# anton-v-bilan/mpeg1video-decoder-webgl

Hardware: AMD Instinct MI355X
Metric: 1080p macroblocks/s (higher is better)
Workload: dtype int32/u8

## Files before the change

mpeg1video-decoder-webgl_amd/csrc/leon_kernels.h:

```cpp
#pragma once
#include <hip/hip_runtime.h>
#include <stdint.h>
#include "leon_resize_row.h"


namespace leon {

struct PicDesc {
    const int16_t* coef[4];
    const uint8_t* qscale;
    const uint8_t* intra;
    const uint8_t* repadd;
    const uint8_t* mb_dir;
    const int16_t* mv_fwd;
    const int16_t* mv_bwd;
    uint8_t*       out;
    const uint8_t* ref_fwd;
    const uint8_t* ref_bwd;
    int32_t        type;
    uint32_t       n_entries;
    const uint32_t* grp_off;
    const uint32_t* entries;
    uint8_t*       rgba;
    int32_t        no_planes;
// ... 235 lines not shown
    o.p43 = v2f{fy6, fy6} + v2f{fy7, -fy7};
    return o;
}

__device__ __forceinline__ ColOut butterfly8_col(const int (&X)[8], int n_live)
{
    const int c128 = 128;
    if (n_live <= 2) {
        const int X0 = X[0], X1 = X[1];
        int x4 = div256(mad24k(X1, 473, c128)) - X1;
        int x0 = x4 - div256(mad24k(X1, 362, c128));
        int y7 = -x0 - div256(mad24k(X1, 196, c128));
        return col_final(X0, X1, X0, x4, X0, x0, X0, y7);
    } else if (n_live <= 4) {
        const int X0 = X[0], X1 = X[1], X2 = X[2], X3 = X[3];
        int b7 = X1 + X3;
        int x4 = div256(mad24k(X1, 473, mad24k(X3, 196, c128))) - b7;
        int x0 = x4 - div256(mad24k(X1 - X3, 362, c128));
        int x2 = div256(mad24k(X2, 362, c128)) - X2;
        int y7 = -x0 - div256(mad24k(X3, -473, mad24k(X1, 196, c128)));
        return col_final(X0 + X2, b7, X0 + x2, x4, X0 - x2, x0, X0 - X2, y7);
    } else {
        int b1 = X[4];
        int b3 = X[2] + X[6];
        int b4 = X[5] - X[3];
        int tmp1 = X[1] + X[7];
        int tmp2 = X[3] + X[5];
        int b6 = X[1] - X[7];
        int b7 = tmp1 + tmp2;
        int m0 = X[0];
        int x4 = div256(mad24k(b6, 473, mad24k(b4, -196, c128))) - b7;
        int x0 = x4 - div256(mad24k(tmp1 - tmp2, 362, c128));
        int x1 = m0 - b1;
        int x2 = div256(mad24k(X[2] - X[6], 362, c128)) - b3;
        int x3 = m0 + b1;
        int y7 = -x0 - div256(mad24k(b4, 473, mad24k(b6, 196, c128)));
        return col_final(x3 + b3, b7, x1 + x2, x4, x1 - x2, x0, x3 - b3, y7);
    }
}

__device__ __forceinline__ int dequant_any(int X, int qO, int pm, int nim, int lo2048, int hi2047)
{
    const int sg = sign3(X);
    int x2 = (X << 1) + (sg & nim);
    int t = mul24_asm(x2, qO);
    int f = t >> 4;
    int z;
    asm("v_med3_i32 %0, %1, 0, 1" : "=v"(z) : "v"(f));
    f = (f - z) | (sg & 1);
    asm("v_med3_i32 %0, %1, %2, %3" : "=v"(f) : "v"(f), "s"(lo2048), "v"(hi2047));
    return __mul24(f, pm);
}

__device__ __forceinline__ int cvt_floor(float x)
{
    int d;
    asm("v_cvt_flr_i32_f32 %0, %1" : "=v"(d) : "v"(x));
    return d;
}

__device__ __forceinline__ int handoff16(int w)
{
    int r = (int)(short)w;
    if (w >= 65536) r = (w & 255) - 256;
    if (w < -65536) r = w & 255;
    return r;
}


__device__ __forceinline__ uint32_t avg4_u8x4(uint32_t a, uint32_t b, uint32_t c, uint32_t d)
{
    const uint32_t X = __builtin_amdgcn_lerp(a, b, c ^ d);
    const uint32_t y = __builtin_amdgcn_lerp(c, d, 0u);
    return __builtin_amdgcn_lerp(X, y, 0x01010101u);
}

__device__ __forceinline__ uint32_t ref_px_clamped(const LEON_GLOBAL uint8_t* ref, uint32_t row_off, int W, int x)
{
    int t = min(max(x >> 2, 0), (W >> 2) - 1);
    return ldg<uint8_t>(ref, row_off + (uint32_t)(4 * t + (x & 3)));
}

typedef v3u U3 __attribute__((aligned(4)));

struct RefRows {
    uint32_t l0, l1, l2;
    uint32_t m0, m1, m2;
    uint32_t s;
    uint32_t oh;
};

__device__ __forceinline__ void gather9_slow(const LEON_GLOBAL uint8_t* ref, uint32_t row_off, int W, int px,
                                             uint32_t& a0, uint32_t& a1, uint32_t& a2)
{
    uint32_t lo = 0, hi = 0;
#pragma unroll 1
    for (int k = 0; k < 4; k++) {
        lo |= ref_px_clamped(ref, row_off, W, px + k) << (8 * k);
        hi |= ref_px_clamped(ref, row_off, W, px + 4 + k) << (8 * k);
    }
    a0 = lo;
    a1 = hi;
    a2 = ref_px_clamped(ref, row_off, W, px + 8);
}

__device__ __forceinline__ int clamp_med3(int v, int hi)
{
    int d;
    asm("v_med3_i32 %0, %1, 0, %2" : "=v"(d) : "v"(v), "s"(hi));
    return d;
}

__device__ __forceinline__ RefRows fetch_rows(const LEON_GLOBAL uint8_t* ref, int W, int H, int y,
                                              int px, int ay, int oh, int ov, bool in_pic, bool last_row, bool use)
{
    const int yy = y + ay;
    const uint32_t r0 = (uint32_t)__mul24(clamp_med3(yy, H - 1), W);
    const uint32_t r1 = r0 + ((uint32_t)yy < (uint32_t)(H - 1) ? (uint32_t)W : 0u);
    RefRows R;
    R.oh = (uint32_t)oh;
    R.m0 = R.m1 = R.m2 = 0;
    if (in_pic) {
        R.s = (uint32_t)px & 3u;
        uint32_t xo = (uint32_t)px & ~3u;
        const __amdgpu_buffer_rsrc_t rs = buf_rsrc((const void*)ref);
        const v3u a = __builtin_amdgcn_raw_buffer_load_b96(rs, (int)(use ? r0 + xo : kOobBit), 0, 0);
        const v3u c = __builtin_amdgcn_raw_buffer_load_b96(rs, (int)(use && last_row && ov ? r1 + xo : kOobBit), 0, 0);
        R.l0 = a.x; R.l1 = a.y; R.l2 = a.z;
        R.m0 = c.x; R.m1 = c.y; R.m2 = c.z;
    } else {
        R.s = 0;
        gather9_slow(ref, r0, W, px, R.l0, R.l1, R.l2);
        if (last_row && ov) gather9_slow(ref, r1, W, px, R.m0, R.m1, R.m2);
    }
    return R;
}

__device__ __forceinline__ void finish_rows(RefRows& R, int ov, bool last_row, int lane, const RefRows* below = nullptr)
{
    const int src = (ov ? ((lane + 8) & 63) : lane) << 2;
    const uint32_t n0 = (uint32_t)__builtin_amdgcn_ds_bpermute(src, (int)R.l0);
    const uint32_t n1 = (uint32_t)__builtin_amdgcn_ds_bpermute(src, (int)R.l1);
    const uint32_t n2 = (uint32_t)__builtin_amdgcn_ds_bpermute(src, (int)R.l2);
    if (below) {
        const uint32_t b0 = (uint32_t)__builtin_amdgcn_ds_bpermute(src, (int)below->l0);
        const uint32_t b1 = (uint32_t)__builtin_amdgcn_ds_bpermute(src, (int)below->l1);
        const uint32_t b2 = (uint32_t)__builtin_amdgcn_ds_bpermute(src, (int)below->l2);
        const bool wrap = last_row && ov;
        R.m0 = wrap ? b0 : n0; R.m1 = wrap ? b1 : n1; R.m2 = wrap ? b2 : n2;
        return;
    }
    if (!(last_row && ov)) { R.m0 = n0; R.m1 = n1; R.m2 = n2; }
}

__device__ __forceinline__ v2u predict8(const RefRows& R)
{
    uint32_t a0 = __builtin_amdgcn_alignbyte(R.l1, R.l0, R.s);
    uint32_t a1 = __builtin_amdgcn_alignbyte(R.l2, R.l1, R.s);
    uint32_t a2 = __builtin_amdgcn_alignbyte(0u, R.l2, R.s);
    uint32_t c0 = __builtin_amdgcn_alignbyte(R.m1, R.m0, R.s);
    uint32_t c1 = __builtin_amdgcn_alignbyte(R.m2, R.m1, R.s);
    uint32_t c2 = __builtin_amdgcn_alignbyte(0u, R.m2, R.s);
    uint32_t b0 = __builtin_amdgcn_alignbyte(a1, a0, R.oh);
    uint32_t b1 = __builtin_amdgcn_alignbyte(a2, a1, R.oh);
    uint32_t d0 = __builtin_amdgcn_alignbyte(c1, c0, R.oh);
    uint32_t d1 = __builtin_amdgcn_alignbyte(c2, c1, R.oh);
    v2u p;
    p.x = avg4_u8x4(a0, b0, c0, d0);
    p.y = avg4_u8x4(a1, b1, c1, d1);
    return p;
}

template <int M>
__device__ __forceinline__ uint32_t pred_x256(uint32_t pred)
{
    uint32_t d;
    asm("v_perm_b32 %0, 0, %1, %2" : "=v"(d) : "v"(pred), "s"(0x0c0c000cu | ((uint32_t)M << 8)));
    return d;
}


struct Display {
    char* stash;
    int side;
    char* apark;
    const char* lut;
    uint8_t* planes;
    const struct FrameOut* fo;
};
static constexpr int kAlphaNone = 0, kAlphaPark = 1, kAlphaTake = 2;

template <int I>
__device__ __forceinline__ uint32_t byte_shl(uint32_t v, uint32_t sh)
{
    uint32_t d;
    if constexpr (I == 0) asm("v_lshlrev_b32_sdwa %0, %1, %2 dst_sel:DWORD dst_unused:UNUSED_PAD src0_sel:DWORD src1_sel:BYTE_0" : "=v"(d) : "v"(sh), "v"(v));
    else if constexpr (I == 1) asm("v_lshlrev_b32_sdwa %0, %1, %2 dst_sel:DWORD dst_unused:UNUSED_PAD src0_sel:DWORD src1_sel:BYTE_1" : "=v"(d) : "v"(sh), "v"(v));
    else if constexpr (I == 2) asm("v_lshlrev_b32_sdwa %0, %1, %2 dst_sel:DWORD dst_unused:UNUSED_PAD src0_sel:DWORD src1_sel:BYTE_2" : "=v"(d) : "v"(sh), "v"(v));
    else asm("v_lshlrev_b32_sdwa %0, %1, %2 dst_sel:DWORD dst_unused:UNUSED_PAD src0_sel:DWORD src1_sel:BYTE_3" : "=v"(d) : "v"(sh), "v"(v));
    return d;
}

struct ChromaTerms { int r, g, b; };
template <int I>
__device__ __forceinline__ ChromaTerms chroma_terms(const char* lut, uint32_t cb2, uint32_t cr2, uint32_t three)
{
    const v2u rc = *reinterpret_cast<const v2u*>(lut + 1024 + byte_shl<I>(cr2, three));
    const v2u bc = *reinterpret_cast<const v2u*>(lut + 3072 + byte_shl<I>(cb2, three));
    return ChromaTerms{(int)rc.x, (int)(rc.y + bc.y), (int)bc.x};
}
template <int I>
__device__ __forceinline__ uint32_t rgba_px(const char* lut, uint32_t y4, const ChromaTerms& c, int a_fixed, uint32_t two)
{
    const int ys = *reinterpret_cast<const int*>(lut + byte_shl<I>(y4, two));
    uint32_t px;
    asm("v_ashr_pk_u8_i32 %0, %1, %2, %3" : "=v"(px) : "v"(ys + c.r), "v"(ys + c.g), "n"(kLutShift));
    asm("v_ashr_pk_u8_i32 %0, %1, %2, %3 op_sel:[0,0,0,1]" : "+v"(px) : "v"(ys + c.b), "v"(a_fixed), "n"(kLutShift));
    return px;
}
template <bool ALPHA>
// ... 50 lines not shown
#pragma unroll
        for (int i = 0; i < 8; i++) o |= *reinterpret_cast<const uint16_t*>(cp + i * 128);
        live[h] = lanes_nonzero((int)o);
        const uint32_t pos = __builtin_amdgcn_mbcnt_hi((uint32_t)(live[h] >> 32), __builtin_amdgcn_mbcnt_lo((uint32_t)live[h], n_before));
        if (o != 0u) *reinterpret_cast<uint8_t*>(ids + pos) = (uint8_t)(tag + (uint32_t)lane + 64u * h);
        n_before += (uint32_t)__builtin_popcountll(live[h]);
    }
    return n_before;
}

template <bool PAIR, bool TLDS = true>
__device__ __forceinline__ void column_pass(char* tile0, uint32_t tile_step, const char* ids, const char* qtab, uint32_t n_cols, int qia0, int qia1, int lane,
                                            uint32_t qreg = 0u)
{
    int lo2048 = -2048, hi2047 = 2047;
    asm("" : "+s"(lo2048), "+v"(hi2047));
#pragma unroll 1
    for (uint32_t base = 0; base < n_cols; base += 64u) {
        const uint32_t k = base + (uint32_t)lane;
        const bool act = k < n_cols;
        uint32_t id = *reinterpret_cast<const uint8_t*>(ids + k);
        id = act ? id : 0u;
        char* colp = tile0 + ((id & 0x47u) << 4) + ((id >> 2) & 14u);
        if constexpr (PAIR) colp += (id >> 7) * tile_step;
        int X[8];
#pragma unroll
        for (int i = 0; i < 8; i++) X[i] = *reinterpret_cast<const short*>(colp + i * 128);
        int bq = __builtin_amdgcn_ds_bpermute((int)((id & 7u) << 2), qia0);
        if constexpr (PAIR) {
            const int bq1 = __builtin_amdgcn_ds_bpermute((int)((id & 7u) << 2), qia1);
            bq = (id & 128u) ? bq1 : bq;
        }
        const bool bia = bq >= 256;
        const uint32_t qv = (uint32_t)bq & 31u;
        v2u msel, pm8;
        if constexpr (TLDS) {
            const char* const qt = qtab + (id & 56u);
            msel = *reinterpret_cast<const v2u*>(qt + (bia ? 0 : 64));
            pm8 = *reinterpret_cast<const v2u*>(qt + 128);
        } else {
            const int qo = (int)((id & 56u) + (bia ? 0u : 64u)), po = (int)((id & 56u) + 128u);
            msel.x = (uint32_t)__builtin_amdgcn_ds_bpermute(qo, (int)qreg);
            msel.y = (uint32_t)__builtin_amdgcn_ds_bpermute(qo + 4, (int)qreg);
            pm8.x = (uint32_t)__builtin_amdgcn_ds_bpermute(po, (int)qreg);
            pm8.y = (uint32_t)__builtin_amdgcn_ds_bpermute(po + 4, (int)qreg);
        }
        int nim = bia ? 0 : -1;
        asm("" : "+v"(nim));
        const bool dc_lane = bia && (id & 56u) == 0u;
        uint64_t nz[8];
#pragma unroll
        for (int i = 0; i < 8; i++) nz[i] = lanes_nonzero(X[i]);
        const int dc = X[0];
        int rows_live = 1;
#pragma unroll
        for (int i = 0; i < 8; i++) {
            if (nz[i] != 0) {
                rows_live = i + 1;
                int P = (int)(((i < 4 ? pm8.x : pm8.y) >> (8 * (i & 3))) & 255u);
                const int qO = (int)__umul24(qv, ((i < 4 ? msel.x : msel.y) >> (8 * (i & 3))) & 255u);
                X[i] = dequant_any(X[i], qO, P, nim, lo2048, hi2047);
            }
        }
        if (dc_lane) X[0] = dc * 256;
        const ColOut co = butterfly8_col(X, rows_live);
        const v2f k04 = {0.4f, 0.4f};
        const v2f s07 = co.p07 * k04, s16 = co.p16 * k04, s52 = co.p52 * k04, s43 = co.p43 * k04;
        int wi[8] = {cvt_floor(s07.x), cvt_floor(s16.x), cvt_floor(s52.y), cvt_floor(s43.y),
                     cvt_floor(s43.x), cvt_floor(s52.x), cvt_floor(s16.y), cvt_floor(s07.y)};
        const float mx = fmaxf(fmaxf(fmaxf(fabsf(s07.x), fabsf(s16.x)), fmaxf(fabsf(s52.y), fabsf(s43.y))),
                               fmaxf(fmaxf(fabsf(s43.x), fabsf(s52.x)), fmaxf(fabsf(s16.y), fabsf(s07.y))));
        if (mx >= 32768.0f) {
#pragma unroll
            for (int n = 0; n < 8; n++) wi[n] = handoff16(wi[n]);
        }
        if (act) {
#pragma unroll
            for (int n = 0; n < 8; n++) *reinterpret_cast<short*>(colp + n * 128) = (short)wi[n];
        }
    }
}

struct MbCarry { uint32_t flags; };
static constexpr int kCarryNone = 0, kCarryLeave = 1, kCarryTake = 2;

template <int TYPE_, bool SPARSE_> struct PlainLuma {
    static constexpr int TYPE = TYPE_, AMODE = kAlphaNone, CARRY = kCarryNone, LAYOUT = 0, OUT = kOutRgba; static constexpr bool SPARSE = SPARSE_, CHROMA = false, DISPLAY = false, BACK = false;
};
template <int TYPE, bool SPARSE> struct PlainChroma : PlainLuma<TYPE, SPARSE> { static constexpr bool CHROMA = true; };
template <int TYPE, bool SPARSE, int LAYOUT_, int OUT_> struct DisplayChroma : PlainChroma<TYPE, SPARSE> {
    static constexpr int CARRY = kCarryLeave, LAYOUT = LAYOUT_, OUT = OUT_; static constexpr bool DISPLAY = true;
};
template <int TYPE, bool SPARSE, int OUT_> struct DisplayLuma : PlainLuma<TYPE, SPARSE> {
    static constexpr int CARRY = kCarryTake, OUT = OUT_; static constexpr bool DISPLAY = true;
};
template <int TYPE, bool SPARSE, int OUT> struct YuvaAPart : DisplayLuma<TYPE, SPARSE, OUT> { static constexpr int AMODE = kAlphaPark; };
template <int TYPE, bool SPARSE, int OUT> struct YuvaYPart : DisplayLuma<TYPE, SPARSE, OUT> { static constexpr int AMODE = kAlphaTake; };
template <int TYPE, int OUT> struct PairBackHalf : DisplayLuma<TYPE, false, OUT> { static constexpr int LAYOUT = 1; static constexpr bool BACK = true; };

struct TaskArgs {
    bool alpha = false;
    char* tile = nullptr;
    uint64_t live[2] = {0, 0};
    uint32_t qreg = 0u;
};

template <int LAYOUT>
__device__ __forceinline__ void column_front(const PicDesc& pd, char* lds, char* tile, int lane, int qia, uint32_t qreg, uint64_t (&live)[2])
{
    const uint32_t n_cols = scan_tile(tile, lds + Lay<LAYOUT>::slots, lane, 0u, 0u, live);
    wave_sync();
    column_pass<false, Lay<LAYOUT>::tables_in_lds>(tile, 0u, lds + Lay<LAYOUT>::slots, Lay<LAYOUT>::tables_in_lds ? lds + kOffQtab : reinterpret_cast<const char*>(pd.qt),
                                                   n_cols, qia, qia, lane, qreg);
    wave_sync();
}

template <typename V>
__device__ __forceinline__ void recon_task(const PicDesc& pd, const Geom& G, int Rt, int g, char* lds, int lane, Display dsp, MbCarry& carry, const TaskArgs& args = TaskArgs())
{
    constexpr int TYPE = V::TYPE, AMODE = V::AMODE, CARRY = V::CARRY, LAYOUT = V::LAYOUT, OUT = V::OUT;
    constexpr bool CHROMA = V::CHROMA, SPARSE = V::SPARSE, DISPLAY = V::DISPLAY, BACK = V::BACK;
    static_assert(!BACK || (LAYOUT == 1 && CARRY == kCarryTake), "a back half runs on the two-tile layout behind the chroma part");
    const bool alpha = AMODE == kAlphaPark || args.alpha;
    char* const tile = BACK ? args.tile : lds;
    const int W = CHROMA ? G.cw >> 1 : G.cw;
    const int H = CHROMA ? G.ch >> 1 : G.ch;
    const int bw = W >> 3;
    const uint32_t ysz = (uint32_t)G.cw * (uint32_t)G.ch;
    const uint32_t a_off = !CHROMA && alpha ? ysz + (ysz >> 1) : 0u;
    const int hi3 = lane >> 3, lo3 = lane & 7;

    const int Qld = g * 8 + lo3;
    const bool ld_ok = Qld < bw;
    const int b = lo3;
    const int Qb = g * 8 + b;
    const bool valid = Qb < bw;
    const int Qs = valid ? Qb : bw - 1;
    const int R0 = CHROMA ? Rt : 2 * Rt;
    const uint32_t coef_voff = (2u * ((uint32_t)__mul24(8 * R0 + hi3, W) + (uint32_t)(8 * Qld))) | (ld_ok ? 0u : kOobBit);
    const uint32_t half_step = CHROMA ? 0u : 8u * (uint32_t)W;
    uint32_t ent_first[2] = {0u, 0u}, ent_start[2] = {0u, 0u}, ent_count[2] = {0u, 0u};
    const __amdgpu_buffer_rsrc_t ent_rs = __builtin_amdgcn_make_buffer_rsrc(
        (void*)(SPARSE ? pd.entries : nullptr), 0, SPARSE ? (int)(pd.n_entries * 4u) : 0, 0x00020000);
    if constexpr (SPARSE) {
        const uint32_t nY = 2u * (uint32_t)G.tasksY, nC = (uint32_t)G.tasksC;
        const uint32_t gid0 = CHROMA ? nY + (uint32_t)(Rt * G.gC + g) : (uint32_t)(2 * Rt * G.gY + g) + (alpha ? nY + 2u * nC : 0u);
        const uint32_t gid1 = CHROMA ? gid0 + nC : gid0 + (uint32_t)G.gY;
        const LEON_GLOBAL uint32_t* go = gptr(pd.grp_off);
        const uint32_t gid[2] = {gid0, gid1};
#pragma unroll
        for (int h = 0; h < 2; h++) {
            const uint32_t s0 = go[gid[h]], e0 = go[gid[h] + 1];
            ent_start[h] = s0;
            ent_count[h] = e0 > s0 ? min(e0 - s0, 512u) : 0u;
            ent_first[h] = (uint32_t)__builtin_amdgcn_raw_buffer_load_b32(
                ent_rs, (int)(((s0 + (uint32_t)lane) * 4u) | ((uint32_t)lane < ent_count[h] ? 0u : kOobBit)), 0, kAuxStreamOnce);
        }
    } else if constexpr (!BACK) {
        wait_lds_all();
        __builtin_amdgcn_wave_barrier();
        coef_rows_to_lds(pd.coef[CHROMA ? 1 : (alpha ? 3 : 0)], lds, coef_voff, 0u);
        coef_rows_to_lds(pd.coef[CHROMA ? 2 : (alpha ? 3 : 0)], lds + kLdsHalf, coef_voff, 2u * half_step);
    }
    const uint32_t mb = (uint32_t)(CHROMA ? Rt * G.mbw + Qs : Rt * G.mbw + (Qs >> 1));
    uint32_t mf = 0, mk = 0, flags;
    if constexpr (CARRY == kCarryTake) {
        const int src = (4 * dsp.side + (lo3 >> 1)) << 2;
        flags = (uint32_t)__builtin_amdgcn_ds_bpermute(src, (int)carry.flags);
        if (TYPE != 1) mf = *reinterpret_cast<const uint32_t*>(lds + Lay<LAYOUT>::carry + src);
        if (TYPE == 3) mk = *reinterpret_cast<const uint32_t*>(lds + Lay<LAYOUT>::carry + 32 + src);
    } else {
        flags = (uint32_t)(ldg<uint8_t>(gptr(pd.qscale), mb) & 31) | (ldg<uint8_t>(gptr(pd.intra), mb) != 0 ? 256u : 0u);
        if (TYPE != 1) {
            flags |= ldg<uint8_t>(gptr(pd.repadd), mb) >= 128 ? 512u : 0u;
            mf = ldg<uint32_t>(gptr(pd.mv_fwd), mb * 4);
        }
        if (TYPE == 3) {
            mk = ldg<uint32_t>(gptr(pd.mv_bwd), mb * 4);
            flags |= (uint32_t)(ldg<uint8_t>(gptr(pd.mb_dir), mb) & 3) << 10;
        }
        if constexpr (CARRY == kCarryLeave) {
            carry.flags = flags;
            if (TYPE != 1) *reinterpret_cast<uint32_t*>(lds + Lay<LAYOUT>::carry + ((lane & 7) << 2)) = mf;
            if (TYPE == 3) *reinterpret_cast<uint32_t*>(lds + Lay<LAYOUT>::carry + 32 + ((lane & 7) << 2)) = mk;
        }
    }
    const int q = (int)(flags & 31u);
    const bool ia = (flags & 256u) != 0u;
    const int x0 = 8 * Qs;
    bool nopred = false;
    int pxA = 0, ayA = 0, ohA = 0, ovA = 0, pxB = 0, ayB = 0, ohB = 0, ovB = 0;
    bool inA = true, inB = true, usef = true, useb = true;
    if (TYPE != 1) {
        nopred = (flags & 512u) != 0u;
        if (TYPE == 3) {
            const int dir = (int)(flags >> 10) & 3;
            usef = (dir & 1) != 0;
            useb = (dir & 2) != 0;
            nopred = nopred || dir == 0;
            if (!usef) mf = 0;
            if (!useb) mk = 0;
        }
        const int fh = (int)(short)(mf & 0xffff), fv = (int)mf >> 16;
        const int bh = (int)(short)(mk & 0xffff), bv = (int)mk >> 16;
        {
            int h = CHROMA ? fh / 2 : fh, v = CHROMA ? fv / 2 : fv;
            pxA = x0 + (h >> 1); ohA = h & 1; ayA = v >> 1; ovA = v & 1;
            inA = (uint32_t)pxA < (uint32_t)(W - 7 - ohA);
        }
        if (TYPE == 3) {
            int h = CHROMA ? bh / 2 : bh, v = CHROMA ? bv / 2 : bv;
            pxB = x0 + (h >> 1); ohB = h & 1; ayB = v >> 1; ovB = v & 1;
            inB = (uint32_t)pxB < (uint32_t)(W - 7 - ohB);
        }
    }
    const bool useA = usef && !nopred, useB = useb && !nopred;
    inA = inA || !useA;
    inB = inB || !useB;
    const int qia = q | (ia ? 256 : 0);

    const uint32_t out_voff = ((uint32_t)__mul24(8 * R0 + hi3, W) + (uint32_t)x0) | (valid ? 0u : kOobBit);
    RefRows rfh[2], rbh[2];
    const bool any_f = TYPE != 3 || __builtin_amdgcn_ballot_w64(useA) != 0;
    const bool any_b = TYPE == 3 && __builtin_amdgcn_ballot_w64(useB) != 0;
    if constexpr (!SPARSE && !BACK) wait_vmem_all();
    if (TYPE != 1) {
#pragma unroll
        for (int h = 0; h < 2; h++) {
            const int Rh = CHROMA ? Rt : 2 * Rt + h;
            const uint32_t po = CHROMA ? (h == 0 ? ysz : ysz + (ysz >> 2)) : a_off;
            const bool ninth = hi3 == 7 && (CHROMA || h == 1);
            if (any_f) rfh[h] = fetch_rows(gptr(pd.ref_fwd) + po, W, H, 8 * Rh + hi3, pxA, ayA, ohA, ovA, inA, ninth, useA);
            if (TYPE == 3 && any_b) rbh[h] = fetch_rows(gptr(pd.ref_bwd) + po, W, H, 8 * Rh + hi3, pxB, ayB, ohB, ovB, inB, ninth, useB);
        }
    }

    if constexpr (SPARSE) {
        *reinterpret_cast<v4i*>(lds + lane * 16) = v4i{0, 0, 0, 0};
        *reinterpret_cast<v4i*>(lds + kLdsHalf + lane * 16) = v4i{0, 0, 0, 0};
        wave_sync();
#pragma unroll
        for (int h = 0; h < 2; h++) {
            uint32_t e = ent_first[h];
            if (e != 0u) *reinterpret_cast<short*>(lds + h * kLdsHalf + ((e >> 16) & 1022u)) = (short)e;
#pragma unroll 1
            for (uint32_t k = 64u; k < ent_count[h]; k += 64u) {
                const uint32_t idx = k + (uint32_t)lane;
                e = (uint32_t)__builtin_amdgcn_raw_buffer_load_b32(
                    ent_rs, (int)(((ent_start[h] + idx) * 4u) | (idx < ent_count[h] ? 0u : kOobBit)), 0, kAuxStreamOnce);
                if (e != 0u) *reinterpret_cast<short*>(lds + h * kLdsHalf + ((e >> 16) & 1022u)) = (short)e;
            }
        }
    }
    wave_sync();

    uint64_t live[2] = {args.live[0], args.live[1]};
    if constexpr (!BACK) column_front<LAYOUT>(pd, lds, tile, lane, qia, args.qreg, live);

#pragma unroll
    for (int half = 0; half < 2; half++) {
        const uint32_t plane_off = CHROMA ? (half == 0 ? ysz : ysz + (ysz >> 2)) : a_off;
        RefRows rf = rfh[half], rb = rbh[half];
        int t[8];
        const uint64_t colbits = live[half];
        if (colbits == 0) {
#pragma unroll
            for (int m = 0; m < 8; m++) t[m] = 128;
        } else {
            const int cols_live = 8 - (__builtin_clzll(colbits | 1ull) >> 3);
            const v4u wv = *reinterpret_cast<const v4u*>(tile + half * kLdsHalf + hi3 * 128 + lo3 * 16);
            const v2f k25 = {2.5f, 2.5f};
            const v2f a = v2f{(float)(short)(wv.x & 0xffffu), (float)((int)wv.x >> 16)} * k25;
            const int Y0 = (int)a.x + 128, Y1 = (int)a.y;
            if (cols_live <= 2) {
                butterfly8_lo2(Y0, Y1, t);
            } else {
                const v2f bb = v2f{(float)(short)(wv.y & 0xffffu), (float)((int)wv.y >> 16)} * k25;
                if (cols_live <= 4) {
                    butterfly8_lo4(Y0, Y1, (int)bb.x, (int)bb.y, t);
                } else {
                    const v2f cc = v2f{(float)(short)(wv.z & 0xffffu), (float)((int)wv.z >> 16)} * k25;
                    const v2f dd = v2f{(float)(short)(wv.w & 0xffffu), (float)((int)wv.w >> 16)} * k25;
                    const int Y[8] = {Y0, Y1, (int)bb.x, (int)bb.y, (int)cc.x, (int)cc.y, (int)dd.x, (int)dd.y};
                    butterfly8(Y, t);
                }
            }
            if (TYPE != 1) {
#pragma unroll
                for (int m = 0; m < 8; m++) t[m] += (t[m] >> 31) & 255;
            }
        }

        if (TYPE != 1) {
            v2u pred = {0u, 0u};
            if (any_f) {
                finish_rows(rf, ovA, hi3 == 7, lane, !CHROMA && half == 0 ? &rfh[1] : nullptr);
                pred = predict8(rf);
            }
            if (TYPE == 3) {
                v2u pb = {0u, 0u};
                if (any_b) {
                    finish_rows(rb, ovB, hi3 == 7, lane, !CHROMA && half == 0 ? &rbh[1] : nullptr);
                    pb = predict8(rb);
                }
                v2u pf = usef ? pred : pb;
                pb = useb ? pb : pred;
                pred.x = __builtin_amdgcn_lerp(pf.x, pb.x, 0x01010101u);
                pred.y = __builtin_amdgcn_lerp(pf.y, pb.y, 0x01010101u);
            }
            if (nopred) pred = v2u{0u, 0u};
            t[0] += pred_x256<0>(pred.x);
            t[1] += pred_x256<1>(pred.x);
            t[2] += pred_x256<2>(pred.x);
            t[3] += pred_x256<3>(pred.x);
            t[4] += pred_x256<0>(pred.y);
            t[5] += pred_x256<1>(pred.y);
// ... 60 lines not shown
    if (TYPE == 3) __builtin_amdgcn_s_setprio(0);
    const int qiaL = __builtin_amdgcn_ds_bpermute((lo3 >> 1) << 2, (int)carry.flags) & 0x11f;
    const int qiaR = __builtin_amdgcn_ds_bpermute((4 + (lo3 >> 1)) << 2, (int)carry.flags) & 0x11f;
    wait_vmem_all();
    wave_sync();
    TaskArgs left{false, lds}, right{false, tileR};
    uint32_t n_cols = scan_tile(lds, lds + Lay<1>::slots, lane, 0u, 0u, left.live);
    if (has_right) n_cols = scan_tile(tileR, lds + Lay<1>::slots, lane, 128u, n_cols, right.live);
    wave_sync();
    column_pass<true, false>(lds, (uint32_t)kOffTileR, lds + Lay<1>::slots, nullptr, n_cols, qiaL, qiaR, lane, qreg);
    wave_sync();
    dsp.side = 0;
    recon_task<PairBackHalf<TYPE, OUT>>(pd, G, Rt, 2 * gc, lds, lane, dsp, carry, left);
    if (has_right) {
        dsp.side = 1;
        recon_task<PairBackHalf<TYPE, OUT>>(pd, G, Rt, 2 * gc + 1, lds, lane, dsp, carry, right);
    }
}

__device__ __forceinline__ void stage_tables(const QTables* __restrict__ Tg, char* lds, int lane)
{
    const __amdgpu_buffer_rsrc_t rs = __builtin_amdgcn_make_buffer_rsrc((void*)Tg, 0, 256, 0x00020000);
    if (lane < 48) __builtin_amdgcn_raw_ptr_buffer_load_lds(rs, (__attribute__((address_space(3))) void*)(lds + kOffQtab), 4, lane * 4, 0, 0, 0);
}

__device__ __forceinline__ int xcd_remap(int bid, int n)
{
    int q = n >> 3, r = n & 7;
    int x = bid & 7, j = bid >> 3;
    return x * q + min(x, r) + j;
}

template <int TYPE>
__device__ __forceinline__ void pic_of_wg(const Geom& G, int wg, int& pic, int& twg)
{
    if (TYPE == 3) {
        const int half = wg >> 1;
        const int pair = div_inv(half, G.inv_wg_per_pic);
        twg = half - pair * G.wg_per_pic;
        pic = 2 * pair + (wg & 1);
    } else {
        pic = div_inv(wg, G.inv_wg_per_pic);
        twg = wg - pic * G.wg_per_pic;
    }
}

template <int TYPE, bool SPARSE>
__device__ __forceinline__ void recon_dispatch(const PicDesc& pd, const Geom& G, int t, char* lds, int lane)
{
    const Display none{nullptr, 0};
    MbCarry own{};
    if (t < G.tasksY) {
        int Rt = div_inv(t, G.inv_gY), g = t - Rt * G.gY;
        recon_task<PlainLuma<TYPE, SPARSE>>(pd, G, Rt, g, lds, lane, none, own);
    } else if (t < G.tasksY + G.tasksC) {
        t -= G.tasksY;
        int Rt = div_inv(t, G.inv_gC), g = t - Rt * G.gC;
        recon_task<PlainChroma<TYPE, SPARSE>>(pd, G, Rt, g, lds, lane, none, own);
    } else {
        t -= G.tasksY + G.tasksC;
        int Rt = div_inv(t, G.inv_gY), g = t - Rt * G.gY;
        recon_task<PlainLuma<TYPE, SPARSE>>(pd, G, Rt, g, lds, lane, none, own, TaskArgs{true});
    }
}

template <int TYPE, bool SPARSE>
__global__ __launch_bounds__(kReconMaxThreads) void k_recon(const PicDesc* __restrict__ descs, Geom G,
                                               const Tables* __restrict__ T)
{
    extern __shared__ __attribute__((aligned(16))) char smem[];
    const int wave = __builtin_amdgcn_readfirstlane(threadIdx.x >> 6);
    const int lane = threadIdx.x & 63;
    const int wg = xcd_remap(blockIdx.x, G.n_wg);
    int pic, twg;
    pic_of_wg<TYPE>(G, wg, pic, twg);
    const int t = twg * kWavesPerWG + wave;
    if (t >= G.tasks_per_pic || pic >= G.n_pics) return;
    char* lds = smem + wave * kLdsPerWave;
    const PicDesc& pd = descs[pic];
    stage_tables(pd.qt, lds, lane);
    recon_dispatch<TYPE, SPARSE>(pd, G, t, lds, lane);
}

template <int TYPE, bool SPARSE, bool ALPHA, int OUT = kOutRgba>
__device__ __forceinline__ bool display_task(const PicDesc* __restrict__ descs, const Geom& G, int pic, int t, char* lds, int lane, const char* lut, bool first,
                                             const FrameOut* fo = nullptr)
{
    constexpr bool kPair = pair_task(TYPE, SPARSE, ALPHA);
    const bool live = t < G.tasks_per_pic && pic < G.n_pics;
    const PicDesc& pd = descs[live ? pic : 0];
    const int Rt = div_inv(t, G.inv_gC), gc = t - Rt * G.gC;
    Display dsp{lds + (kPair ? Lay<1>::stash : Lay<0>::stash), 0, lds + kLdsPerWaveDisplay, lut, nullptr, fo};
    if constexpr (OUT != kOutRgba) dsp.planes = fo->frames[live ? pic : 0];
    if constexpr (!kPair) {
        if (!first) { wait_lds_all(); __builtin_amdgcn_wave_barrier(); }
        stage_tables(pd.qt, lds, lane);
    }
    MbCarry carry{};
    uint32_t qreg = 0u;
    if constexpr (kPair) qreg = ldg<uint32_t>(gptr(pd.qt), (uint32_t)lane * 4u);
    const TaskArgs tables{false, nullptr, {0, 0}, qreg};
    if (live) recon_task<DisplayChroma<TYPE, SPARSE, kPair ? 1 : 0, OUT>>(pd, G, Rt, gc, lds, lane, dsp, carry, tables);
    if (first) {
        if (!live) wait_vmem_all();
        if constexpr (OUT != kOutYcbcr) __syncthreads();
    }
    if (!live) return false;
    if constexpr (kPair) {
        recon_luma_pair<TYPE, OUT>(pd, G, Rt, gc, lds, lane, dsp, carry, 2 * gc + 1 < G.gY, qreg);
        return true;
    }
    dsp.side = 0;
    if constexpr (ALPHA) {
        recon_task<YuvaAPart<TYPE, SPARSE, OUT>>(pd, G, Rt, 2 * gc, lds, lane, dsp, carry);
        recon_task<YuvaYPart<TYPE, SPARSE, OUT>>(pd, G, Rt, 2 * gc, lds, lane, dsp, carry);
    } else {
        recon_task<DisplayLuma<TYPE, SPARSE, OUT>>(pd, G, Rt, 2 * gc, lds, lane, dsp, carry);
    }
    if (2 * gc + 1 < G.gY) {
        dsp.side = 1;
        if constexpr (ALPHA) {
            recon_task<YuvaAPart<TYPE, SPARSE, OUT>>(pd, G, Rt, 2 * gc + 1, lds, lane, dsp, carry);
            recon_task<YuvaYPart<TYPE, SPARSE, OUT>>(pd, G, Rt, 2 * gc + 1, lds, lane, dsp, carry);
        } else {
            recon_task<DisplayLuma<TYPE, SPARSE, OUT>>(pd, G, Rt, 2 * gc + 1, lds, lane, dsp, carry);
        }
    }
    return true;
}

template <int TYPE, bool SPARSE, bool ALPHA = false>
__global__ __launch_bounds__(kReconMaxThreads) __attribute__((amdgpu_waves_per_eu(TYPE == 3 && !ALPHA ? 7 : 4)))
void k_recon_display(const PicDesc* __restrict__ descs, Geom G,
                                                                    const Tables* __restrict__ T)
{
    extern __shared__ __attribute__((aligned(16))) char smem[];
    if (TYPE == 3 && !SPARSE && !ALPHA) __builtin_amdgcn_s_setprio(3);
    const int wave = __builtin_amdgcn_readfirstlane(threadIdx.x >> 6);
    const int lane0 = threadIdx.x & 63;
    const int wg = xcd_remap(blockIdx.x, G.n_wg);
    int pic, twg;
    pic_of_wg<TYPE>(G, wg, pic, twg);
    const int wpw = (int)(blockDim.x >> 6);
    __shared__ __attribute__((aligned(16))) int32_t lut_s[kLdsLut / 4];
    static_assert(kLdsLut % 1024 == 0, "whole chunks");
    const __amdgpu_buffer_rsrc_t lrs = __builtin_amdgcn_make_buffer_rsrc((void*)T->rgba_lut, 0, kLdsLut, 0x00020000);
    for (int c = wave; c < kLdsLut / 1024; c += wpw)
        __builtin_amdgcn_raw_ptr_buffer_load_lds(lrs, (__attribute__((address_space(3))) void*)(reinterpret_cast<char*>(lut_s) + c * 1024), 16,
                                                 (int)(lane0 * 16u), c * 1024, 0, 0);
    char* lds = smem + wave * display_strip_bytes(TYPE, SPARSE, ALPHA);
    display_task<TYPE, SPARSE, ALPHA>(descs, G, pic, twg * wpw + wave, lds, lane0, reinterpret_cast<const char*>(lut_s), true);
}


template <int TYPE, bool SPARSE, bool ALPHA, int OUT>
__global__ __launch_bounds__(kReconMaxThreads) __attribute__((amdgpu_waves_per_eu(TYPE == 3 && !ALPHA ? 7 : (TYPE == 2 && ALPHA && OUT == kOutBoth ? 8 : 4))))
void k_recon_display_out(const PicDesc* __restrict__ descs, Geom G, const Tables* __restrict__ T, FrameOut fo)
{
    extern __shared__ __attribute__((aligned(16))) char smem[];
    if (TYPE == 3 && !SPARSE && !ALPHA) __builtin_amdgcn_s_setprio(3);
    const int wave = __builtin_amdgcn_readfirstlane(threadIdx.x >> 6);
    const int lane0 = threadIdx.x & 63;
    const int wg = xcd_remap(blockIdx.x, G.n_wg);
    int pic, twg;
    pic_of_wg<TYPE>(G, wg, pic, twg);
    const int wpw = (int)(blockDim.x >> 6);
    __shared__ __attribute__((aligned(16))) int32_t lut_s[kLdsLut / 4];
    if constexpr (OUT == kOutBoth) {
        const __amdgpu_buffer_rsrc_t lrs = __builtin_amdgcn_make_buffer_rsrc((void*)T->rgba_lut, 0, kLdsLut, 0x00020000);
        for (int c = wave; c < kLdsLut / 1024; c += wpw)
            __builtin_amdgcn_raw_ptr_buffer_load_lds(lrs, (__attribute__((address_space(3))) void*)(reinterpret_cast<char*>(lut_s) + c * 1024), 16,
                                                     (int)(lane0 * 16u), c * 1024, 0, 0);
    }
    char* lds = smem + wave * display_strip_bytes(TYPE, SPARSE, ALPHA);
    display_task<TYPE, SPARSE, ALPHA, OUT>(descs, G, pic, twg * wpw + wave, lds, lane0, OUT == kOutBoth ? reinterpret_cast<const char*>(lut_s) : nullptr, true, &fo);
}

struct CropGeom {
    int32_t cw, ch, fw, fh;
    int32_t cwid;
    uint32_t slot_stride_lo, slot_stride_hi;
    int32_t alpha;
};
__global__ __launch_bounds__(kRgbaBlock) void k_planes_crop(const uint8_t* __restrict__ slots, const int32_t* __restrict__ src_slots, FrameOut fo, CropGeom G)
{
    const int plane = blockIdx.y;
    if (plane == 3 && !G.alpha) return;
    const bool luma = plane == 0 || plane == 3;
    const uint32_t piece = luma ? 16u : 8u;
    const uint32_t pw = (uint32_t)(luma ? G.fw : G.cwid), ph = (uint32_t)(luma ? G.fh : fo.chroma_height);
    const uint32_t per_row = (pw + piece - 1) / piece;
    const uint32_t idx = blockIdx.x * (uint32_t)blockDim.x + threadIdx.x;
    if (idx >= per_row * ph) return;
    const uint32_t y = idx / per_row, x = (idx - y * per_row) * piece;
    const uint32_t ysz = (uint32_t)G.cw * (uint32_t)G.ch;
    const uint32_t src_w = luma ? (uint32_t)G.cw : (uint32_t)G.cw >> 1;
    const uint32_t src_plane = plane == 0 ? 0u : plane == 1 ? ysz : plane == 2 ? ysz + (ysz >> 2) : ysz + (ysz >> 1);
    const size_t stride = join64(G.slot_stride_lo, G.slot_stride_hi);
    const uint8_t* src = slots + (size_t)src_slots[blockIdx.z] * stride + src_plane + (size_t)y * src_w + x;
    uint8_t* dst = fo.frames[blockIdx.z] + (plane == 0 ? 0u : plane == 1 ? fo.cb_off : plane == 2 ? fo.cr_off : fo.a_off)
                 + (size_t)y * (luma ? fo.luma_stride : fo.chroma_stride) + x;
    if (luma) *reinterpret_cast<uint4*>(dst) = *reinterpret_cast<const uint4*>(src);
    else *reinterpret_cast<uint2*>(dst) = *reinterpret_cast<const uint2*>(src);
}


struct RgbaGeom {
    int32_t cw, ch, fw, fh;
    int32_t cols, rows;
    int32_t n;
    int32_t flavour;
    uint32_t slot_stride_lo, slot_stride_hi;
    uint32_t inv_cols4;
};

__device__ __forceinline__ uint32_t u8_clamped(double x)
{
    double t = x + 6755399441055744.0;
    int i = __double2loint(t);
    return (uint32_t)med3i(i, 0, 255);
}

__global__ __launch_bounds__(kRgbaBlock) void k_rgba_twin(const uint8_t* __restrict__ slots, const int32_t* __restrict__ slot_ids,
                                                   uint8_t* __restrict__ rgba, RgbaGeom G)
{
    const int col = blockIdx.x * blockDim.x + threadIdx.x;
    const int row = blockIdx.y;
    const int f = blockIdx.z;
    if (col >= G.cols) return;
    const size_t stride = join64(G.slot_stride_lo, G.slot_stride_hi);
    const uint8_t* Y = slots + (size_t)slot_ids[f] * stride;
    const uint8_t* Cb = Y + (size_t)G.cw * G.ch;
    const uint8_t* Cr = Cb + ((size_t)G.cw * G.ch >> 2);
    uint8_t* dst = rgba + (size_t)f * G.fw * G.fh * 4;
    const int odd = G.fw & 1;
    const int hw = G.cw >> 1;
    const int yi1 = row * (2 * G.cw - odd) + 2 * col;
    const int yi2 = yi1 + G.cw;
    const int ci = row * hw + col;
    const size_t d1 = 4 * ((size_t)row * (2 * G.fw - odd) + 2 * col);
    const size_t d2 = d1 + 4 * (size_t)G.fw;
    const double yuvr = (double)Cr[ci] - 128.0, yuvb = (double)Cb[ci] - 128.0;
    const double r = yuvr * 1.59603;
    const double g = (-0.81297 * yuvr) - (0.39176 * yuvb);
    const double b = yuvb * 2.01723;
    uint32_t px[4];
    const int yidx[4] = {yi1, yi1 + 1, yi2, yi2 + 1};
#pragma unroll
    for (int k = 0; k < 4; k++) {
        double ys = ((double)Y[yidx[k]] - 16.0) * 1.16438;
        px[k] = u8_clamped(r + ys) | (u8_clamped(g + ys) << 8) | (u8_clamped(b + ys) << 16) | 0xff000000u;
    }
    *reinterpret_cast<uint32_t*>(dst + d1) = px[0];
    *reinterpret_cast<uint32_t*>(dst + d1 + 4) = px[1];
    *reinterpret_cast<uint32_t*>(dst + d2) = px[2];
    *reinterpret_cast<uint32_t*>(dst + d2 + 4) = px[3];
}

// ... 842 lines not shown
```

Baseline: 2.302 billion.

## Precompute in-picture luma motion offsets in chroma pass and pin kernel args in SGPRs

The chroma pass now checks, per wave, whether every macroblock's motion vector keeps the luma 16x16 reference inside the picture. If so, it passes a packed offset word (base offset, sub-word shift, half-pel bits) to the luma pass, which then uses a simpler fetch path without clamping or per-lane coordinate maths. The change also loads group offsets as a single 2-word load made uniform, hoists the picture descriptor fetch into the kernel, and uses empty asm constraints to keep kernel arguments and descriptor fields in scalar registers. The aim is fewer VALU instructions and less register pressure in the luma reconstruction, at the cost of extra ballots and more complex carry encoding.

New measurement: 2.263 billion. -1.7%, worse.

```diff
diff --git a/mpeg1video-decoder-webgl_amd/csrc/leon_kernels.h b/mpeg1video-decoder-webgl_amd/csrc/leon_kernels.h
--- a/mpeg1video-decoder-webgl_amd/csrc/leon_kernels.h
+++ b/mpeg1video-decoder-webgl_amd/csrc/leon_kernels.h
@@ -341,6 +341,7 @@
 }
 
 typedef v3u U3 __attribute__((aligned(4)));
+typedef v2u U2 __attribute__((aligned(4)));
 
 struct RefRows {
     uint32_t l0, l1, l2;
@@ -395,6 +396,19 @@
     return R;
 }
 
+__device__ __forceinline__ RefRows fetch_rows_inside(const LEON_GLOBAL uint8_t* ref, int W, uint32_t off, uint32_t s, uint32_t oh, int ov, bool last_row, bool use)
+{
+    RefRows R;
+    R.oh = oh;
+    R.s = s;
+    const __amdgpu_buffer_rsrc_t rs = buf_rsrc((const void*)ref);
+    const v3u a = __builtin_amdgcn_raw_buffer_load_b96(rs, (int)(use ? off : kOobBit), 0, 0);
+    const v3u c = __builtin_amdgcn_raw_buffer_load_b96(rs, (int)(use && last_row && ov ? off + (uint32_t)W : kOobBit), 0, 0);
+    R.l0 = a.x; R.l1 = a.y; R.l2 = a.z;
+    R.m0 = c.x; R.m1 = c.y; R.m2 = c.z;
+    return R;
+}
+
 __device__ __forceinline__ void finish_rows(RefRows& R, int ov, bool last_row, int lane, const RefRows* below = nullptr)
 {
     const int src = (ov ? ((lane + 8) & 63) : lane) << 2;
@@ -611,20 +625,29 @@
 }
 
 struct MbCarry { uint32_t flags; };
+static constexpr uint32_t kCarryInsideF = 1u << 12, kCarryInsideB = 1u << 13;
+static constexpr uint32_t kInsideOffMask = (1u << 26) - 1u;
+__device__ __forceinline__ uint32_t inside_word(uint32_t mv, int mbx, int mby, int W, int H, bool& in)
+{
+    const int h = (int)(short)(mv & 0xffff), v = (int)mv >> 16;
+    const int x = 16 * mbx + (h >> 1), y = 16 * mby + (v >> 1), oh = h & 1, ov = v & 1;
+    in = (uint32_t)x < (uint32_t)(W - 15 - oh) && (uint32_t)y < (uint32_t)(H - 15 - ov);
+    return ((uint32_t)__mul24(y, W) + ((uint32_t)x & ~3u)) | ((uint32_t)x & 3u) << 26 | (uint32_t)oh << 28 | (uint32_t)ov << 29;
+}
 static constexpr int kCarryNone = 0, kCarryLeave = 1, kCarryTake = 2;
 
 template <int TYPE_, bool SPARSE_> struct PlainLuma {
-    static constexpr int TYPE = TYPE_, AMODE = kAlphaNone, CARRY = kCarryNone, LAYOUT = 0, OUT = kOutRgba; static constexpr bool SPARSE = SPARSE_, CHROMA = false, DISPLAY = false, BACK = false;
+    static constexpr int TYPE = TYPE_, AMODE = kAlphaNone, CARRY = kCarryNone, LAYOUT = 0, OUT = kOutRgba; static constexpr bool SPARSE = SPARSE_, CHROMA = false, DISPLAY = false, BACK = false, INSIDE = false;
 };
 template <int TYPE, bool SPARSE> struct PlainChroma : PlainLuma<TYPE, SPARSE> { static constexpr bool CHROMA = true; };
-template <int TYPE, bool SPARSE, int LAYOUT_, int OUT_> struct DisplayChroma : PlainChroma<TYPE, SPARSE> {
-    static constexpr int CARRY = kCarryLeave, LAYOUT = LAYOUT_, OUT = OUT_; static constexpr bool DISPLAY = true;
+template <int TYPE, bool SPARSE, int LAYOUT_, int OUT_, bool INSIDE_> struct DisplayChroma : PlainChroma<TYPE, SPARSE> {
+    static constexpr int CARRY = kCarryLeave, LAYOUT = LAYOUT_, OUT = OUT_; static constexpr bool DISPLAY = true, INSIDE = INSIDE_ && TYPE != 1;
 };
 template <int TYPE, bool SPARSE, int OUT_> struct DisplayLuma : PlainLuma<TYPE, SPARSE> {
-    static constexpr int CARRY = kCarryTake, OUT = OUT_; static constexpr bool DISPLAY = true;
-};
-template <int TYPE, bool SPARSE, int OUT> struct YuvaAPart : DisplayLuma<TYPE, SPARSE, OUT> { static constexpr int AMODE = kAlphaPark; };
-template <int TYPE, bool SPARSE, int OUT> struct YuvaYPart : DisplayLuma<TYPE, SPARSE, OUT> { static constexpr int AMODE = kAlphaTake; };
+    static constexpr int CARRY = kCarryTake, OUT = OUT_; static constexpr bool DISPLAY = true, INSIDE = TYPE != 1;
+};
+template <int TYPE, bool SPARSE, int OUT> struct YuvaAPart : DisplayLuma<TYPE, SPARSE, OUT> { static constexpr int AMODE = kAlphaPark; static constexpr bool INSIDE = false; };
+template <int TYPE, bool SPARSE, int OUT> struct YuvaYPart : DisplayLuma<TYPE, SPARSE, OUT> { static constexpr int AMODE = kAlphaTake; static constexpr bool INSIDE = false; };
 template <int TYPE, int OUT> struct PairBackHalf : DisplayLuma<TYPE, false, OUT> { static constexpr int LAYOUT = 1; static constexpr bool BACK = true; };
 
 struct TaskArgs {
@@ -648,7 +671,7 @@
 __device__ __forceinline__ void recon_task(const PicDesc& pd, const Geom& G, int Rt, int g, char* lds, int lane, Display dsp, MbCarry& carry, const TaskArgs& args = TaskArgs())
 {
     constexpr int TYPE = V::TYPE, AMODE = V::AMODE, CARRY = V::CARRY, LAYOUT = V::LAYOUT, OUT = V::OUT;
-    constexpr bool CHROMA = V::CHROMA, SPARSE = V::SPARSE, DISPLAY = V::DISPLAY, BACK = V::BACK;
+    constexpr bool CHROMA = V::CHROMA, SPARSE = V::SPARSE, DISPLAY = V::DISPLAY, BACK = V::BACK, INSIDE = V::INSIDE;
     static_assert(!BACK || (LAYOUT == 1 && CARRY == kCarryTake), "a back half runs on the two-tile layout behind the chroma part");
     const bool alpha = AMODE == kAlphaPark || args.alpha;
     char* const tile = BACK ? args.tile : lds;
@@ -679,7 +702,16 @@
         const uint32_t gid[2] = {gid0, gid1};
 #pragma unroll
         for (int h = 0; h < 2; h++) {
-            const uint32_t s0 = go[gid[h]], e0 = go[gid[h] + 1];
+            uint32_t s0, e0;
+            if constexpr (DISPLAY) {
+                uint32_t at = gid[h] * 4u;
+                asm("" : "+v"(at));
+                const v2u se = ldg<U2>(go, at);
+                s0 = (uint32_t)__builtin_amdgcn_readfirstlane((int)se.x);
+                e0 = (uint32_t)__builtin_amdgcn_readfirstlane((int)se.y);
+            } else {
+                s0 = go[gid[h]]; e0 = go[gid[h] + 1];
+            }
             ent_start[h] = s0;
             ent_count[h] = e0 > s0 ? min(e0 - s0, 512u) : 0u;
             ent_first[h] = (uint32_t)__builtin_amdgcn_raw_buffer_load_b32(
@@ -709,9 +741,20 @@
             flags |= (uint32_t)(ldg<uint8_t>(gptr(pd.mb_dir), mb) & 3) << 10;
         }
         if constexpr (CARRY == kCarryLeave) {
+            uint32_t cf = mf, ck = mk;
+            if constexpr (INSIDE) {
+                const bool np = (flags & 512u) != 0u || (TYPE == 3 && (flags & (3u << 10)) == 0u);
+                bool in;
+                const uint32_t wf = inside_word(mf, Qs, Rt, G.cw, G.ch, in);
+                if (__builtin_amdgcn_ballot_w64(!in && !np && (TYPE != 3 || (flags & (1u << 10)) != 0u)) == 0) { cf = wf; flags |= kCarryInsideF; }
+                if constexpr (TYPE == 3) {
+                    const uint32_t wk = inside_word(mk, Qs, Rt, G.cw, G.ch, in);
+                    if (__builtin_amdgcn_ballot_w64(!in && !np && (flags & (2u << 10)) != 0u) == 0) { ck = wk; flags |= kCarryInsideB; }
+                }
+            }
             carry.flags = flags;
-            if (TYPE != 1) *reinterpret_cast<uint32_t*>(lds + Lay<LAYOUT>::carry + ((lane & 7) << 2)) = mf;
-            if (TYPE == 3) *reinterpret_cast<uint32_t*>(lds + Lay<LAYOUT>::carry + 32 + ((lane & 7) << 2)) = mk;
+            if (TYPE != 1) *reinterpret_cast<uint32_t*>(lds + Lay<LAYOUT>::carry + ((lane & 7) << 2)) = cf;
+            if (TYPE == 3) *reinterpret_cast<uint32_t*>(lds + Lay<LAYOUT>::carry + 32 + ((lane & 7) << 2)) = ck;
         }
     }
     const int q = (int)(flags & 31u);
@@ -720,6 +763,9 @@
     bool nopred = false;
     int pxA = 0, ayA = 0, ohA = 0, ovA = 0, pxB = 0, ayB = 0, ohB = 0, ovB = 0;
     bool inA = true, inB = true, usef = true, useb = true;
+    uint32_t offA = 0u, sA = 0u, offB = 0u, sB = 0u;
+    const uint32_t uflags = INSIDE && CARRY == kCarryTake ? (uint32_t)__builtin_amdgcn_readfirstlane((int)flags) : 0u;
+    const bool insF = (uflags & kCarryInsideF) != 0u, insB = (uflags & kCarryInsideB) != 0u;
     if (TYPE != 1) {
         nopred = (flags & 512u) != 0u;
         if (TYPE == 3) {
@@ -727,20 +773,27 @@
             usef = (dir & 1) != 0;
             useb = (dir & 2) != 0;
             nopred = nopred || dir == 0;
-            if (!usef) mf = 0;
-            if (!useb) mk = 0;
-        }
-        const int fh = (int)(short)(mf & 0xffff), fv = (int)mf >> 16;
-        const int bh = (int)(short)(mk & 0xffff), bv = (int)mk >> 16;
-        {
+            if (!usef && !insF) mf = 0;
+            if (!useb && !insB) mk = 0;
+        }
+        const uint32_t in_row = (uint32_t)__mul24(hi3, W) + 8u * (uint32_t)(b & 1);
+        if (insF) {
+            offA = (mf & kInsideOffMask) + in_row; sA = (mf >> 26) & 3u; ohA = (int)(mf >> 28) & 1; ovA = (int)(mf >> 29) & 1;
+        } else {
+            const int fh = (int)(short)(mf & 0xffff), fv = (int)mf >> 16;
             int h = CHROMA ? fh / 2 : fh, v = CHROMA ? fv / 2 : fv;
             pxA = x0 + (h >> 1); ohA = h & 1; ayA = v >> 1; ovA = v & 1;
             inA = (uint32_t)pxA < (uint32_t)(W - 7 - ohA);
         }
         if (TYPE == 3) {
-            int h = CHROMA ? bh / 2 : bh, v = CHROMA ? bv / 2 : bv;
-            pxB = x0 + (h >> 1); ohB = h & 1; ayB = v >> 1; ovB = v & 1;
-            inB = (uint32_t)pxB < (uint32_t)(W - 7 - ohB);
+            if (insB) {
+                offB = (mk & kInsideOffMask) + in_row; sB = (mk >> 26) & 3u; ohB = (int)(mk >> 28) & 1; ovB = (int)(mk >> 29) & 1;
+            } else {
+                const int bh = (int)(short)(mk & 0xffff), bv = (int)mk >> 16;
+                int h = CHROMA ? bh / 2 : bh, v = CHROMA ? bv / 2 : bv;
+                pxB = x0 + (h >> 1); ohB = h & 1; ayB = v >> 1; ovB = v & 1;
+                inB = (uint32_t)pxB < (uint32_t)(W - 7 - ohB);
+            }
         }
     }
     const bool useA = usef && !nopred, useB = useb && !nopred;
@@ -759,8 +812,11 @@
             const int Rh = CHROMA ? Rt : 2 * Rt + h;
             const uint32_t po = CHROMA ? (h == 0 ? ysz : ysz + (ysz >> 2)) : a_off;
             const bool ninth = hi3 == 7 && (CHROMA || h == 1);
-            if (any_f) rfh[h] = fetch_rows(gptr(pd.ref_fwd) + po, W, H, 8 * Rh + hi3, pxA, ayA, ohA, ovA, inA, ninth, useA);
-            if (TYPE == 3 && any_b) rbh[h] = fetch_rows(gptr(pd.ref_bwd) + po, W, H, 8 * Rh + hi3, pxB, ayB, ohB, ovB, inB, ninth, useB);
+            const uint32_t half_rows = h ? 8u * (uint32_t)W : 0u;
+            if (any_f) rfh[h] = insF ? fetch_rows_inside(gptr(pd.ref_fwd) + po, W, offA + half_rows, sA, (uint32_t)ohA, ovA, ninth, useA)
+                                     : fetch_rows(gptr(pd.ref_fwd) + po, W, H, 8 * Rh + hi3, pxA, ayA, ohA, ovA, inA, ninth, useA);
+            if (TYPE == 3 && any_b) rbh[h] = insB ? fetch_rows_inside(gptr(pd.ref_bwd) + po, W, offB + half_rows, sB, (uint32_t)ohB, ovB, ninth, useB)
+                                                  : fetch_rows(gptr(pd.ref_bwd) + po, W, H, 8 * Rh + hi3, pxB, ayB, ohB, ovB, inB, ninth, useB);
         }
     }
 
@@ -987,16 +1043,63 @@
     recon_dispatch<TYPE, SPARSE>(pd, G, t, lds, lane);
 }
 
+__device__ __forceinline__ void raise_priority(int& workgroup) { asm("s_setprio 3" : "+s"(workgroup)); }
+typedef uint8_t* const LEON_GLOBAL* FramesPtr;
+template <bool SPARSE>
+__device__ __forceinline__ void hold_args(Geom& G, const LEON_GLOBAL PicDesc*& descs, const Tables*& T, int& wpw, int& workgroup)
+{
+    uint64_t size = join64((uint32_t)G.cw, (uint32_t)G.ch), groups = join64((uint32_t)G.gY, (uint32_t)G.gC), frame = join64((uint32_t)G.fw, (uint32_t)G.fh),
+             pics = join64((uint32_t)G.n_pics, (uint32_t)G.n_wg), tasks = join64((uint32_t)G.tasksY, (uint32_t)G.tasksC);
+    if constexpr (SPARSE)
+        asm("" : "+s"(size), "+s"(groups), "+s"(frame), "+s"(pics), "+s"(tasks), "+s"(G.mbw), "+s"(G.tasks_per_pic), "+s"(G.wg_per_pic), "+s"(G.inv_wg_per_pic),
+                 "+s"(G.inv_gC), "+s"(descs), "+s"(T), "+s"(wpw), "+s"(workgroup));
+    else
+        asm("" : "+s"(size), "+s"(groups), "+s"(frame), "+s"(pics), "+s"(G.mbw), "+s"(G.tasks_per_pic), "+s"(G.wg_per_pic), "+s"(G.inv_wg_per_pic),
+                 "+s"(G.inv_gC), "+s"(descs), "+s"(T), "+s"(wpw), "+s"(workgroup));
+    G.cw = (int32_t)size; G.ch = (int32_t)(size >> 32); G.gY = (int32_t)groups; G.gC = (int32_t)(groups >> 32);
+    G.fw = (int32_t)frame; G.fh = (int32_t)(frame >> 32); G.n_pics = (int32_t)pics; G.n_wg = (int32_t)(pics >> 32);
+    if constexpr (SPARSE) { G.tasksY = (int32_t)tasks; G.tasksC = (int32_t)(tasks >> 32); }
+}
+__device__ __forceinline__ void hold_frame_out(FrameOut& fo, FramesPtr& frames)
+{
+    asm("" : "+s"(frames), "+s"(fo.luma_stride), "+s"(fo.chroma_stride), "+s"(fo.cb_off), "+s"(fo.cr_off), "+s"(fo.a_off), "+s"(fo.chroma_height));
+}
+template <int TYPE, bool SPARSE, bool ALPHA, int OUT>
+__device__ __forceinline__ void hold_desc(PicDesc& d, uint8_t*& planes)
+{
+    asm volatile("" : "+s"(d.qt), "+s"(d.qscale), "+s"(d.intra), "+s"(d.out), "+s"(d.no_planes), "+s"(d.rgba));
+    if constexpr (OUT != kOutRgba) asm volatile("" : "+s"(planes));
+    if constexpr (!SPARSE) {
+        asm volatile("" : "+s"(d.coef[0]), "+s"(d.coef[1]), "+s"(d.coef[2]));
+        if constexpr (ALPHA) asm volatile("" : "+s"(d.coef[3]));
+    } else {
+        asm volatile("" : "+s"(d.n_entries), "+s"(d.grp_off), "+s"(d.entries));
+    }
+    if constexpr (TYPE != 1) asm volatile("" : "+s"(d.repadd), "+s"(d.mv_fwd), "+s"(d.ref_fwd));
+    if constexpr (TYPE == 3) asm volatile("" : "+s"(d.mb_dir), "+s"(d.mv_bwd), "+s"(d.ref_bwd));
+}
+template <int TYPE, bool SPARSE, bool ALPHA, int OUT>
+__device__ __forceinline__ PicDesc fetch_desc(const LEON_GLOBAL PicDesc* descs, const Geom& G, int pic, int t, uint8_t*& planes,
+                                              FramesPtr frames = nullptr)
+{
+    const int at = t < G.tasks_per_pic && pic < G.n_pics ? pic : 0;
+    const LEON_GLOBAL PicDesc& s = descs[at];
+    PicDesc pd{{s.coef[0], s.coef[1], s.coef[2], s.coef[3]}, s.qscale, s.intra, s.repadd, s.mb_dir, s.mv_fwd, s.mv_bwd, s.out, s.ref_fwd, s.ref_bwd,
+               s.type, s.n_entries, s.grp_off, s.entries, s.rgba, s.no_planes, 0, s.qt};
+    planes = nullptr;
+    if constexpr (OUT != kOutRgba) planes = frames[at];
+    hold_desc<TYPE, SPARSE, ALPHA, OUT>(pd, planes);
+    return pd;
+}
+
 template <int TYPE, bool SPARSE, bool ALPHA, int OUT = kOutRgba>
-__device__ __forceinline__ bool display_task(const PicDesc* __restrict__ descs, const Geom& G, int pic, int t, char* lds, int lane, const char* lut, bool first,
-                                             const FrameOut* fo = nullptr)
+__device__ __forceinline__ bool display_task(const PicDesc& pd, const Geom& G, int pic, int t, char* lds, int lane, const char* lut, bool first,
+                                             const FrameOut* fo = nullptr, uint8_t* planes = nullptr)
 {
     constexpr bool kPair = pair_task(TYPE, SPARSE, ALPHA);
     const bool live = t < G.tasks_per_pic && pic < G.n_pics;
-    const PicDesc& pd = descs[live ? pic : 0];
     const int Rt = div_inv(t, G.inv_gC), gc = t - Rt * G.gC;
-    Display dsp{lds + (kPair ? Lay<1>::stash : Lay<0>::stash), 0, lds + kLdsPerWaveDisplay, lut, nullptr, fo};
-    if constexpr (OUT != kOutRgba) dsp.planes = fo->frames[live ? pic : 0];
+    Display dsp{lds + (kPair ? Lay<1>::stash : Lay<0>::stash), 0, lds + kLdsPerWaveDisplay, lut, planes, fo};
     if constexpr (!kPair) {
         if (!first) { wait_lds_all(); __builtin_amdgcn_wave_barrier(); }
         stage_tables(pd.qt, lds, lane);
@@ -1005,7 +1108,7 @@
     uint32_t qreg = 0u;
     if constexpr (kPair) qreg = ldg<uint32_t>(gptr(pd.qt), (uint32_t)lane * 4u);
     const TaskArgs tables{false, nullptr, {0, 0}, qreg};
-    if (live) recon_task<DisplayChroma<TYPE, SPARSE, kPair ? 1 : 0, OUT>>(pd, G, Rt, gc, lds, lane, dsp, carry, tables);
+    if (live) recon_task<DisplayChroma<TYPE, SPARSE, kPair ? 1 : 0, OUT, !ALPHA>>(pd, G, Rt, gc, lds, lane, dsp, carry, tables);
     if (first) {
         if (!live) wait_vmem_all();
         if constexpr (OUT != kOutYcbcr) __syncthreads();
@@ -1036,17 +1139,23 @@
 
 template <int TYPE, bool SPARSE, bool ALPHA = false>
 __global__ __launch_bounds__(kReconMaxThreads) __attribute__((amdgpu_waves_per_eu(TYPE == 3 && !ALPHA ? 7 : 4)))
-void k_recon_display(const PicDesc* __restrict__ descs, Geom G,
-                                                                    const Tables* __restrict__ T)
+void k_recon_display(const PicDesc* __restrict__ descs_, Geom G,
+                                                                    const Tables* __restrict__ T_)
 {
     extern __shared__ __attribute__((aligned(16))) char smem[];
-    if (TYPE == 3 && !SPARSE && !ALPHA) __builtin_amdgcn_s_setprio(3);
+    int bid = (int)blockIdx.x;
+    if (TYPE == 3 && !SPARSE && !ALPHA) raise_priority(bid);
     const int wave = __builtin_amdgcn_readfirstlane(threadIdx.x >> 6);
     const int lane0 = threadIdx.x & 63;
-    const int wg = xcd_remap(blockIdx.x, G.n_wg);
+    const LEON_GLOBAL PicDesc* descs = gptr(descs_);
+    const Tables* T = T_;
+    int wpw = (int)(blockDim.x >> 6);
+    hold_args<SPARSE>(G, descs, T, wpw, bid);
+    const int wg = xcd_remap(bid, G.n_wg);
     int pic, twg;
     pic_of_wg<TYPE>(G, wg, pic, twg);
-    const int wpw = (int)(blockDim.x >> 6);
+    uint8_t* planes;
+    const PicDesc pd = fetch_desc<TYPE, SPARSE, ALPHA, kOutRgba>(descs, G, pic, twg * wpw + wave, planes);
     __shared__ __attribute__((aligned(16))) int32_t lut_s[kLdsLut / 4];
     static_assert(kLdsLut % 1024 == 0, "whole chunks");
     const __amdgpu_buffer_rsrc_t lrs = __builtin_amdgcn_make_buffer_rsrc((void*)T->rgba_lut, 0, kLdsLut, 0x00020000);
@@ -1054,22 +1163,30 @@
         __builtin_amdgcn_raw_ptr_buffer_load_lds(lrs, (__attribute__((address_space(3))) void*)(reinterpret_cast<char*>(lut_s) + c * 1024), 16,
                                                  (int)(lane0 * 16u), c * 1024, 0, 0);
     char* lds = smem + wave * display_strip_bytes(TYPE, SPARSE, ALPHA);
-    display_task<TYPE, SPARSE, ALPHA>(descs, G, pic, twg * wpw + wave, lds, lane0, reinterpret_cast<const char*>(lut_s), true);
+    display_task<TYPE, SPARSE, ALPHA>(pd, G, pic, twg * wpw + wave, lds, lane0, reinterpret_cast<const char*>(lut_s), true);
 }
 
 
 template <int TYPE, bool SPARSE, bool ALPHA, int OUT>
 __global__ __launch_bounds__(kReconMaxThreads) __attribute__((amdgpu_waves_per_eu(TYPE == 3 && !ALPHA ? 7 : (TYPE == 2 && ALPHA && OUT == kOutBoth ? 8 : 4))))
-void k_recon_display_out(const PicDesc* __restrict__ descs, Geom G, const Tables* __restrict__ T, FrameOut fo)
+void k_recon_display_out(const PicDesc* __restrict__ descs_, Geom G, const Tables* __restrict__ T_, FrameOut fo)
 {
     extern __shared__ __attribute__((aligned(16))) char smem[];
-    if (TYPE == 3 && !SPARSE && !ALPHA) __builtin_amdgcn_s_setprio(3);
+    int bid = (int)blockIdx.x;
+    if (TYPE == 3 && !SPARSE && !ALPHA) raise_priority(bid);
     const int wave = __builtin_amdgcn_readfirstlane(threadIdx.x >> 6);
     const int lane0 = threadIdx.x & 63;
-    const int wg = xcd_remap(blockIdx.x, G.n_wg);
+    const LEON_GLOBAL PicDesc* descs = gptr(descs_);
+    FramesPtr frames = gptr(fo.frames);
+    const Tables* T = T_;
+    int wpw = (int)(blockDim.x >> 6);
+    hold_args<SPARSE>(G, descs, T, wpw, bid);
+    hold_frame_out(fo, frames);
+    const int wg = xcd_remap(bid, G.n_wg);
     int pic, twg;
     pic_of_wg<TYPE>(G, wg, pic, twg);
-    const int wpw = (int)(blockDim.x >> 6);
+    uint8_t* planes;
+    const PicDesc pd = fetch_desc<TYPE, SPARSE, ALPHA, OUT>(descs, G, pic, twg * wpw + wave, planes, frames);
     __shared__ __attribute__((aligned(16))) int32_t lut_s[kLdsLut / 4];
     if constexpr (OUT == kOutBoth) {
         const __amdgpu_buffer_rsrc_t lrs = __builtin_amdgcn_make_buffer_rsrc((void*)T->rgba_lut, 0, kLdsLut, 0x00020000);
@@ -1078,7 +1195,7 @@
                                                      (int)(lane0 * 16u), c * 1024, 0, 0);
     }
     char* lds = smem + wave * display_strip_bytes(TYPE, SPARSE, ALPHA);
-    display_task<TYPE, SPARSE, ALPHA, OUT>(descs, G, pic, twg * wpw + wave, lds, lane0, OUT == kOutBoth ? reinterpret_cast<const char*>(lut_s) : nullptr, true, &fo);
+    display_task<TYPE, SPARSE, ALPHA, OUT>(pd, G, pic, twg * wpw + wave, lds, lane0, OUT == kOutBoth ? reinterpret_cast<const char*>(lut_s) : nullptr, true, &fo, planes);
 }
 
 struct CropGeom {
```
